# preon7/2019global

Measured on AMD Instinct MI355X. Metric: Mray/s + ms/frame at 1920x1080, depth 8; %HBM roofline, higher is better.
Workload: dtype f64

## Files before the change

2019global_amd/csrc/gi_wf.hip:

```cpp
#include <hip/hip_runtime.h>

#include <algorithm>
#include <cstdlib>
#include <mutex>
#include <type_traits>

#include "gi.h"
#include "gi_dev.h"
#include "gi_scene.h"

namespace gi {
namespace {

constexpr long long kWfTile = 8;

#ifndef GI_WF_MIN_WAVES_LDS
#define GI_WF_MIN_WAVES_LDS 4
#endif
#ifndef GI_WF_MIN_WAVES
#define GI_WF_MIN_WAVES 3
#endif
#ifndef GI_WF_TAKE
#define GI_WF_TAKE 16
#endif
constexpr size_t kWfSlotBytes = 9 * 256 * sizeof(double);

struct PathId {
    uint64_t key;
    unsigned smp;
    int b;
};
__device__ __forceinline__ void slot_put_u64(double* pl, int f, uint64_t v) { reinterpret_cast<uint64_t*>(pl)[f * 256] = v; }
__device__ __forceinline__ uint64_t slot_get_u64(const double* pl, int f) { return reinterpret_cast<const uint64_t*>(pl)[f * 256]; }

struct WFQ {
    double* r;
    uint2* id;
    long long cap;
};

template <bool ANY, bool PAIR, bool AXIS, bool SH, bool TRI, bool NST, typename NodeP, typename HotP>
__device__ __forceinline__ int wf_trace(float far_r, NodeP W, HotP H, V3 o, V3 d, double tmax, bool act, int* nst, double& t_out,
                                        uint32_t& nnode, uint32_t& nprim, uint32_t& nsteps, int skip = 254) {
    constexpr bool kSkip = std::is_same<NodeP, const XWNode*>::value;
    const F3 of = ray_org32(o, d, far_r);
    const F3 ivf = inv_dir(d);
    const int dmask = (d.x < 0 ? 1 : 0) | (d.y < 0 ? 2 : 0) | (d.z < 0 ? 4 : 0);
    double tb = tmax;
    float tbf = up32(tmax);
    int best = -1;
    uint64_t mlo = 0, mhi = 0;
    int node = 0, level = 0;
    bool raying = false;
    if (act) {
        uint32_t rm;
        if constexpr (kSkip) rm = children_mask<AXIS, true>(W, of, ivf, tbf, dmask, skip);
        else rm = children_mask<AXIS>(W, of, ivf, tbf, dmask);
        lvl_set<SH>(mlo, mhi, 0, rm);
        raying = rm != 0;
    }
    while (raying) {
        ++nsteps;
        const auto* nd = W + node;
        const uint32_t msk = lvl_get<SH>(mlo, mhi, level);
        const int kc = __builtin_ctz(msk);
        lvl_set<SH>(mlo, mhi, level, msk & (msk - 1));
        const int c = kc ^ dmask;
        bool keep = true;
        if (!ANY && !NST && best >= 0) {
            keep = child_hit(nd, c, of, ivf, tbf);
        }
        const int ch = nd->child[c];
        if (keep) {
            if (ch < 0) {
                const int cnt = nd->cnt[c];
                const auto* hp = H + ~ch;
                if constexpr (PAIR) {
                    for (int j = 0; j < cnt; j += 2) {
                        const bool two = j + 1 < cnt;
                        const XHotR r0 = load_hot(hp + j), r1 = load_hot(hp + (two ? j + 1 : j));
                        const double ta = x_prim_t<TRI>(r0.h, o, d, MX_TMIN);
                        const double tq = two ? x_prim_t<TRI>(r1.h, o, d, MX_TMIN) : INFINITY;
                        nprim += two ? 2 : 1;
                        if (ANY) {
                            if ((ta < tmax) | (tq < tmax)) {
                                best = ta < tmax ? r0.h.prim : r1.h.prim;
                                break;
                            }
                        } else {
                            const bool ua = (ta < tb) | ((ta == tb) & (r0.h.prim < best));
                            tb = ua ? ta : tb;
                            best = ua ? r0.h.prim : best;
                            const bool uq = (tq < tb) | ((tq == tb) & (r1.h.prim < best));
                            tb = uq ? tq : tb;
                            best = uq ? r1.h.prim : best;
                            tbf = up32(tb);
                        }
                    }
                } else {
                    XHotR cur = load_hot(hp);
                    for (int j = 0; j < cnt; ++j) {
                        const XHotR rec = cur;
                        if (j + 1 < cnt) cur = load_hot(hp + j + 1);
                        ++nprim;
                        const double t = x_prim_t<TRI>(rec.h, o, d, MX_TMIN);
                        if (ANY) {
                            if (t < tmax) { best = rec.h.prim; break; }
                        } else {
                            const bool u = (t < tb) | ((t == tb) & (rec.h.prim < best));
                            tb = u ? t : tb;
                            best = u ? rec.h.prim : best;
                            tbf = u ? up32(t) : tbf;
                        }
                    }
                }
            } else {
                ++nnode;
                uint32_t cm;
                if constexpr (kSkip) cm = children_mask<AXIS, true>(W + ch, of, ivf, tbf, dmask, skip);
                else cm = children_mask<AXIS>(W + ch, of, ivf, tbf, dmask);
                if (cm) {
                    node = ch;
                    ++level;
                    lvl_set<SH>(mlo, mhi, level, cm);
                    if (NST) nst[level * 256] = ch;
                }
            }
        }
        if (ANY && best >= 0) break;
        uint32_t rest = lvl_get<SH>(mlo, mhi, level);
        if (rest == 0 && level > 0) {
            if constexpr (NST) {
                const uint64_t lm = level >= 8 ? mlo : mlo & ((1ull << (8 * level)) - 1);
                const uint64_t hm = level <= 8 ? 0ull : mhi & ((1ull << (8 * (level - 8))) - 1);
                level = hm ? 8 + (63 - __clzll((long long)hm)) / 8 : lm ? (63 - __clzll((long long)lm)) / 8 : 0;
                rest = lvl_get<SH>(mlo, mhi, level);
                node = level == 0 ? 0 : nst[level * 256];
            } else {
                do {
                    --level;
                    node = level == 0 ? 0 : W[node].parent;
                    rest = lvl_get<SH>(mlo, mhi, level);
                } while (rest == 0 && level > 0);
            }
        }
        raying = rest != 0;
    }
    t_out = tb;
    return best;
}

#ifndef GI_XFLAT_CHUNK
#define GI_XFLAT_CHUNK 0
#endif
#ifndef GI_XFLAT_UNROLL
#define GI_XFLAT_UNROLL 4
#endif
#ifndef GI_XFLAT_LDS
#define GI_XFLAT_LDS 0
#endif
typedef uint32_t u32x8 __attribute__((ext_vector_type(8)));
__device__ __forceinline__ u32x8 flat_rec_uniform(const XFlatLeaf* tab, int k) {
#if GI_XFLAT_LDS
    const int4* q = reinterpret_cast<const int4*>(tab + k);
    const int4 a = q[0], b = q[1];
    return u32x8{(uint32_t)a.x, (uint32_t)a.y, (uint32_t)a.z, (uint32_t)a.w, (uint32_t)b.x, (uint32_t)b.y, (uint32_t)b.z, (uint32_t)b.w};
#else
    return *(const __attribute__((address_space(4))) u32x8*)(uintptr_t)(tab + k);
#endif
}
__device__ __forceinline__ uint32_t flat_pack(uint32_t off, int k, uint32_t w7) { return off | ((uint32_t)k << 16) | ((w7 & 0xFFu) << 24); }
__device__ __forceinline__ bool flat_hit(const XFlatLeaf* r, F3 no, F3 ivf, int sm, float tmax, uint32_t& pk, int k) {
    const int4* q = reinterpret_cast<const int4*>(r);
    const int4 a = q[0], b = q[1];
    const float lx = __int_as_float(a.x), ly = __int_as_float(a.y), lz = __int_as_float(a.z);
    const float hx = __int_as_float(a.w), hy = __int_as_float(b.x), hz = __int_as_float(b.y);
    const float nx = (sm & 1) ? hx : lx, fx = (sm & 1) ? lx : hx;
    const float ny = (sm & 2) ? hy : ly, fy = (sm & 2) ? ly : hy;
    const float nz = (sm & 4) ? hz : lz, fz = (sm & 4) ? lz : hz;
    const float tn = fmaxf(fmaxf(__builtin_fmaf(nx, ivf.x, no.x), __builtin_fmaf(ny, ivf.y, no.y)),
                           fmaxf(__builtin_fmaf(nz, ivf.z, no.z), 0.0f));
    const float tf = fminf(fminf(__builtin_fmaf(fx, ivf.x, no.x), __builtin_fmaf(fy, ivf.y, no.y)),
                           fminf(__builtin_fmaf(fz, ivf.z, no.z), tmax));
    pk = flat_pack((uint32_t)b.z, k, (uint32_t)b.w);
    return tn <= tf;
}
template <bool ANY, bool TRI>
__device__ __forceinline__ int wf_flat(float far_r, const XFlatLeaf* tab, int n, const XHot* H, V3 o, V3 d, double tmax, bool act,
                                       double& t_out, uint32_t& nnode, uint32_t& nprim, uint32_t& nsteps, int skip) {
    const F3 of = ray_org32(o, d, far_r);
    const F3 ivf = inv_dir(d);
    const F3 no = neg_oiv(of, ivf);
    const int sm = iv_signs(ivf);
    const bool sx = (sm & 1) != 0, sy = (sm & 2) != 0, sz = (sm & 4) != 0;
    double tb = tmax;
    float tbf = up32(tmax);
    int best = -1;
    const float tfa = act ? tbf : -1.0f;
    uint32_t m = 0, pk = 0;
    float tn1 = INFINITY, tn2 = INFINITY;
    auto step = [&](const u32x8 w, int k) {
        const float lx = __uint_as_float(w[0]), ly = __uint_as_float(w[1]), lz = __uint_as_float(w[2]);
        const float hx = __uint_as_float(w[3]), hy = __uint_as_float(w[4]), hz = __uint_as_float(w[5]);
        const float ax = __builtin_fmaf(lx, ivf.x, no.x), bx = __builtin_fmaf(hx, ivf.x, no.x);
        const float ay = __builtin_fmaf(ly, ivf.y, no.y), by = __builtin_fmaf(hy, ivf.y, no.y);
        const float az = __builtin_fmaf(lz, ivf.z, no.z), bz = __builtin_fmaf(hz, ivf.z, no.z);
        const float tn = fmaxf(fmaxf(sx ? bx : ax, sy ? by : ay), fmaxf(sz ? bz : az, 0.0f));
        const float tf = fminf(fminf(sx ? ax : bx, sy ? ay : by), fminf(sz ? az : bz, tfa));
        const bool hit = (tn <= tf) & ((int)((w[7] >> 16) & 0xFFu) != skip);
        const uint32_t pkk = flat_pack(w[6], k, w[7]);
        m |= hit ? 1u << k : 0u;
        if (ANY) {
            pk = hit ? pkk : pk;
        } else {
            const float th = hit ? tn : INFINITY;
            pk = th < tn1 ? pkk : pk;
            tn2 = __builtin_amdgcn_fmed3f(tn1, tn2, th);
            tn1 = fminf(tn1, th);
        }
    };
    int k0 = 0;
#if GI_XFLAT_CHUNK
    for (; k0 + 4 <= n; k0 += 4) {
        const u32x8 w0 = flat_rec_uniform(tab, k0), w1 = flat_rec_uniform(tab, k0 + 1);
        const u32x8 w2 = flat_rec_uniform(tab, k0 + 2), w3 = flat_rec_uniform(tab, k0 + 3);
        step(w0, k0);
        step(w1, k0 + 1);
        step(w2, k0 + 2);
        step(w3, k0 + 3);
    }
#pragma unroll 1
#else
#pragma unroll GI_XFLAT_UNROLL
#endif
    for (int k = k0; k < n; ++k) step(flat_rec_uniform(tab, k), k);
    if (act) nnode += (uint32_t)((n * (int)sizeof(XFlatLeaf) + 255) / 256);
    bool go = m != 0;
    if (go) m &= ~(1u << ((pk >> 16) & 0xFFu));
    while (go) {
        ++nsteps;
        const int cnt = (int)(pk >> 24);
        const XHot* hp = H + (pk & 0xFFFFu);
        for (int j = 0; j < cnt; j += 2) {
            const bool two = j + 1 < cnt;
            const XHotR r0 = load_hot(hp + j), r1 = load_hot(hp + (two ? j + 1 : j));
            const double ta = x_prim_t<TRI>(r0.h, o, d, MX_TMIN);
            const double tq = two ? x_prim_t<TRI>(r1.h, o, d, MX_TMIN) : INFINITY;
            nprim += two ? 2 : 1;
            if (ANY) {
                if ((ta < tmax) | (tq < tmax)) {
                    best = ta < tmax ? r0.h.prim : r1.h.prim;
                    break;
                }
            } else {
                const bool ua = (ta < tb) | ((ta == tb) & (r0.h.prim < best));
                tb = ua ? ta : tb;
                best = ua ? r0.h.prim : best;
                const bool uq = (tq < tb) | ((tq == tb) & (r1.h.prim < best));
                tb = uq ? tq : tb;
                best = uq ? r1.h.prim : best;
                tbf = up32(tb);
            }
        }
        go = false;
        if (ANY) {
            if (best < 0 && m != 0) {
                const int k = 31 - __builtin_clz(m);
                m &= ~(1u << k);
                const int4 b = reinterpret_cast<const int4*>(tab + k)[1];
                pk = flat_pack((uint32_t)b.z, k, (uint32_t)b.w);
                go = true;
            }
        } else {
            if (tn2 > tbf) m = 0;
            while (m != 0) {
                const int k = __builtin_ctz(m);
                m &= m - 1;
                if (flat_hit(tab + k, no, ivf, sm, tbf, pk, k)) {
                    go = true;
                    break;
                }
            }
        }
    }
    t_out = tb;
    return best;
}

struct WFArgs {
    const unsigned* list;
    const unsigned* n_list;
    double* part;
    unsigned* take;
    const unsigned* n_in;
    unsigned* n_out;
    unsigned long long u0, u1;
    unsigned s0, ns;
};

struct WFView {
    const XWNode* LW = nullptr;
    const XHot* LH = nullptr;
    const XPrim* XP = nullptr;
    const REnt* EN = nullptr;
    const XFlatLeaf* FT = nullptr;
    int* nst = nullptr;
    double* pl = nullptr;
};
template <bool LDS>
__device__ __forceinline__ WFView wf_stage(const DevScene& sc, int4* lds) {
    WFView v;
    v.XP = sc.xprims;
    v.EN = sc.ents;
    v.FT = sc.xflat;
    if constexpr (LDS) {
        const int nw = sc.n_xwnodes * (int)(sizeof(XWNode) / sizeof(int4));
        const int nh = sc.n_xhot * (int)(sizeof(XHot) / sizeof(int4));
        const int np = sc.n_xprims * (int)(sizeof(XPrim) / sizeof(int4));
        const int ne = sc.n_ents * (int)(sizeof(REnt) / sizeof(int4));
        const int nf = GI_XFLAT_LDS ? sc.n_xflat * (int)(sizeof(XFlatLeaf) / sizeof(int4)) : 0;
        const int4* gw = reinterpret_cast<const int4*>(sc.xwnodes);
        const int4* gh = reinterpret_cast<const int4*>(sc.xhot);
        const int4* gp = reinterpret_cast<const int4*>(sc.xprims);
        const int4* ge = reinterpret_cast<const int4*>(sc.ents);
        const int4* gf = reinterpret_cast<const int4*>(sc.xflat);
        for (int i = threadIdx.x; i < nw; i += blockDim.x) lds[i] = gw[i];
        for (int i = threadIdx.x; i < nh; i += blockDim.x) lds[nw + i] = gh[i];
        for (int i = threadIdx.x; i < np; i += blockDim.x) lds[nw + nh + i] = gp[i];
        for (int i = threadIdx.x; i < ne; i += blockDim.x) lds[nw + nh + np + i] = ge[i];
        for (int i = threadIdx.x; i < nf; i += blockDim.x) lds[nw + nh + np + ne + i] = gf[i];
        __syncthreads();
        v.LW = reinterpret_cast<const XWNode*>(lds);
        v.LH = reinterpret_cast<const XHot*>(lds + nw);
        v.XP = reinterpret_cast<const XPrim*>(lds + nw + nh);
        v.EN = reinterpret_cast<const REnt*>(lds + nw + nh + np);
        if (GI_XFLAT_LDS) v.FT = reinterpret_cast<const XFlatLeaf*>(lds + nw + nh + np + ne);
        v.pl = reinterpret_cast<double*>(lds + nw + nh + np + ne + nf) + threadIdx.x;
    } else {
        v.nst = reinterpret_cast<int*>(lds) + threadIdx.x;
        v.pl = reinterpret_cast<double*>(reinterpret_cast<int*>(lds) + 16 * 256) + threadIdx.x;
    }
    return v;
}

__device__ __forceinline__ V3 wf_primary(const CamDev& cam, const TileMap& m, unsigned ps, int spp, uint64_t seed,
                                         unsigned li, unsigned smp, long long& idx, uint64_t& key) {
    int x = 0, y = 0;
    slot_pixel(m, (long long)(ps >> 6), (int)(ps & 63), idx, x, y);
    y += m.y0;
    if (spp > 1) idx = (long long)li;
    key = mx_key(seed, (uint64_t)y * (uint64_t)m.w + (uint64_t)x);
    double jx = 0.0, jy = 0.0;
    if (spp > 1) {
        jx = mx_u01k(key, smp, 0xFFFF, 0);
        jy = mx_u01k(key, smp, 0xFFFF, 1);
    }
    return primary_dir(cam, (double)x + jx, (double)y + jy);
}
__device__ __forceinline__ bool wf_primary_misses(const DevScene& sc, const CamDev& cam, V3 d0) {
    const F3 iv0 = f3(__builtin_amdgcn_rcpf((float)d0.x), __builtin_amdgcn_rcpf((float)d0.y), __builtin_amdgcn_rcpf((float)d0.z));
    return !root_hit(sc, ray_org32(cam.pos, d0, ray_far_r(sc, cam.pos)), iv0);
}
__device__ __forceinline__ void wf_store(double* part, double* rgb, uint8_t* rgb8, int spp, long long idx, unsigned smp, V3 L) {
    if (spp > 1) {
        double* q = part + 3 * ((size_t)idx * (size_t)spp + (size_t)smp);
        q[0] = L.x; q[1] = L.y; q[2] = L.z;
    } else {
        const double c0 = smin((0.0 + L.x) / 1.0, 1.0), c1 = smin((0.0 + L.y) / 1.0, 1.0), c2 = smin((0.0 + L.z) / 1.0, 1.0);
        if (rgb) { rgb[3 * idx] = c0; rgb[3 * idx + 1] = c1; rgb[3 * idx + 2] = c2; }
        if (rgb8) quantize(c0, c1, c2, rgb8 + 3 * idx);
    }
}

struct WFSegStats {
    uint64_t it_c = 0, ln_c = 0, it_s = 0, ln_s = 0, segs = 0, live = 0, iters = 0;
    uint64_t cyc_c = 0, cyc_s = 0, cyc_sh = 0, cyc_ref = 0, cyc_all = 0;
};
__device__ __forceinline__ void wf_wave_steps(uint32_t n, uint64_t& it, uint64_t& ln) {
    uint32_t mx = n, sm = n;
    for (int off = 32; off > 0; off >>= 1) {
        mx = max(mx, (uint32_t)__shfl_xor(mx, off));
        sm += __shfl_xor(sm, off);
    }
    if ((threadIdx.x & 63) == 0) { it += mx; ln += sm; }
}
template <bool ANY, bool LDS, bool SH, bool TRI, bool CN, bool FLAT>
__device__ __forceinline__ int x_query(const DevScene& sc, const WFView& v, float far_r, const V3& o, const V3& d, double tmax,
                                       bool act, double& t_out, uint32_t& nnode, uint32_t& nprim, uint32_t& st_steps, int skip) {
    if constexpr (FLAT) return wf_flat<ANY, TRI>(far_r, v.FT, sc.n_xflat, v.LH, o, d, tmax, act, t_out, nnode, nprim, st_steps, skip);
    else if constexpr (LDS) return wf_trace<ANY, true, false, SH, TRI, false>(far_r, v.LW, v.LH, o, d, tmax, act, v.nst, t_out, nnode, nprim, st_steps, skip);
    else if constexpr (CN) return wf_trace<ANY, false, false, SH, TRI, true>(far_r, sc.xcnodes, sc.xhot, o, d, tmax, act, v.nst, t_out, nnode, nprim, st_steps);
    else return wf_trace<ANY, false, false, SH, TRI, true>(far_r, sc.xwnodes, sc.xhot, o, d, tmax, act, v.nst, t_out, nnode, nprim, st_steps, skip);
}
__device__ __forceinline__ int x_own_plane(int pg, const V3& pn, const V3& dir, double skip_cos) {
    return (pg < 254 && fabs(dot(dir, pn)) >= skip_cos) ? pg : 254;
}
struct XHitFrame { V3 P, Ld, pn; double ldist; int pg; };
__device__ __forceinline__ XHitFrame x_hit_frame(const WFView& v, const V3& light, const V3& o, const V3& d, bool hit, int best, double t) {
    XHitFrame h{o, v3(0, 0, 1), v3(0, 0, 1), 0.0, 254};
    if (hit) {
        h.P = o + t * d;
        const V3 lv = light - h.P;
        h.ldist = gsqrt(dot(lv, lv));
        h.Ld = normalize(lv);
        const XPrim& px = v.XP[best];
        h.pg = px.pad[0] < 254 ? px.pad[0] : 254;
        h.pn = ld3(px.n);
    }
    return h;
}

template <bool STATS, bool LDS, bool SH, bool TRI, bool CN, bool FLAT, typename KeyF>
__device__ __forceinline__ bool x_segment(const DevScene& sc, const WFView& v, const V3& light, int depth, bool no_shadow, bool act,
                                          const KeyF& id_of, V3& o, V3& d, V3& L, V3& T,
                                          uint32_t& nnode, uint32_t& nprim, uint32_t& nrays, WFSegStats& ws,
                                          double skip_cos = 2.0, int* splane = nullptr, float far_r = INFINITY) {
    uint32_t st_steps = 0;
    uint64_t c0 = STATS ? clock64() : 0;
    bool occl = false;
    double tbest = INFINITY;
    const int skip_c = splane ? *splane : 254;
    const int best = x_query<false, LDS, SH, TRI, CN, FLAT>(sc, v, far_r, o, d, INFINITY, act, tbest, nnode, nprim, st_steps, skip_c);
    if (act) ++nrays;
    if (STATS) {
        wf_wave_steps(st_steps, ws.it_c, ws.ln_c);
        st_steps = 0;
        const uint64_t c1 = clock64();
        ws.cyc_c += c1 - c0;
        c0 = c1;
    }
    const bool hit = act && best >= 0;
    const XHitFrame h = x_hit_frame(v, light, o, d, hit, best, tbest);
    const V3 &P = h.P, &Ld = h.Ld;
    if (!no_shadow) {
        double tdummy;
        const int skip_s = x_own_plane(h.pg, h.pn, Ld, skip_cos);
        occl = x_query<true, LDS, SH, TRI, CN, FLAT>(sc, v, INFINITY, P, Ld, h.ldist, hit, tdummy, nnode, nprim, st_steps, skip_s) >= 0;
        if (STATS) wf_wave_steps(st_steps, ws.it_s, ws.ln_s);
    }
    if (STATS) {
        const uint64_t c1 = clock64();
        ws.cyc_s += c1 - c0;
        c0 = c1;
    }
    {
        L = v3(v.pl[0], v.pl[256], v.pl[512]);
        T = v3(v.pl[768], v.pl[1024], v.pl[1280]);
    }
    bool cont = false;
    if (hit) {
        ++nrays;
        const XPrim& p = v.XP[best];
        V3 N = (TRI || p.kind == 0) ? ld3(p.n) : normalize(P - ld3(p.a));
        N = dot(d, N) < 0 ? N : -N;
        const REnt& e = v.EN[p.ent];
        int32_t tu, tv;
        x_texcoord<TRI>(sc, e, P, tu, tv);
        const V3 tc = texel(ld3(e.color), tu, tv);
        const V3 la = tc * e.shader[0];
        V3 loc = la;
        if (!occl) {
            const V3 ldf = (smax(0.0, dot(N, Ld)) * (tc * 0.5)) * e.shader[1];
            const V3 bis = normalize(normalize(-d) + Ld);
            const double spw = mx_pow(smax(0.0, dot(N, bis)), e.spec_pow);
            const V3 ls = v3(spw, spw, spw) * e.shader[2];
            loc = (la + ldf) + ls;
        }
        L = L + vmul(T, v3(smin(loc.x, 1.0), smin(loc.y, 1.0), smin(loc.z, 1.0)));
        const PathId id = id_of();
        const uint64_t key = id.key;
        const unsigned smp = id.smp;
        const int b = id.b;
        if (b != depth - 1) {
            if (e.refl > 0.0 && mx_u01k(key, smp, b, 4) < e.refl) {
                d = normalize(d - N * (2.0 * dot(d, N)));
                cont = true;
            } else {
                T = vmul(T, tc * 0.5);
                if (!((T.x == 0.0) & (T.y == 0.0) & (T.z == 0.0))) {
                    double sx, sy, r2;
                    mx_disk(mx_u01k(key, smp, b, 2), mx_u01k(key, smp, b, 3), sx, sy, r2);
                    const double sz = gsqrt(1.0 - r2);
                    const double sg = N.z >= 0.0 ? 1.0 : -1.0;
                    const double aa = -1.0 / (sg + N.z);
                    const double bb = N.x * N.y * aa;
                    const V3 bt1 = v3(1.0 + sg * N.x * N.x * aa, sg * bb, -sg * N.x);
                    const V3 bt2 = v3(bb, sg + N.y * N.y * aa, -N.y);
                    d = normalize((bt1 * sx + bt2 * sy) + N * sz);
                    cont = true;
                }
            }
            o = P;
        }
        if (cont) {
            v.pl[0] = L.x; v.pl[256] = L.y; v.pl[512] = L.z;
            v.pl[768] = T.x; v.pl[1024] = T.y; v.pl[1280] = T.z;
            if (splane) *splane = x_own_plane(h.pg, h.pn, d, skip_cos);
        }
    }
    if (STATS) ws.cyc_sh += clock64() - c0;
    return cont;
}

template <bool STATS, bool LDS, bool W4, bool SH, bool TRI, bool CN, bool FLAT>
__global__ __launch_bounds__(256, (LDS && W4) ? GI_WF_MIN_WAVES_LDS : GI_WF_MIN_WAVES) void k_wf_bounce(
    DevScene sc, CamDev cam, V3 light, TileMap m, int spp, int depth, uint64_t seed, int b, double* rgb, uint8_t* rgb8,
    unsigned long long* stats, WFArgs a, WFQ qin, WFQ qout, int xflags) {
    unsigned n_in;
    if (b == 0) {
        const unsigned long long tot = (unsigned long long)*a.n_list * (unsigned long long)a.ns;
        n_in = (unsigned)(min(tot, a.u1) > a.u0 ? min(tot, a.u1) - a.u0 : 0ull);
    } else {
        n_in = *a.n_in;
    }
    if (*(volatile unsigned*)a.take >= n_in) return;
    extern __shared__ int4 lds_dyn[];
    const WFView v = wf_stage<LDS>(sc, lds_dyn);
    const bool no_shadow = (xflags & XF_NO_SHADOW) != 0;
    const int lane = threadIdx.x & 63;
    uint32_t nnode = 0, nprim = 0, nrays = 0, nres = 0, npx = 0;
    const long long qc = qin.cap, oc = qout.cap;
    const unsigned take = (unsigned)max(1u, min((unsigned)GI_WF_TAKE, n_in / (64u * 8u * (gridDim.x * (blockDim.x >> 6)))));
    unsigned base = 0, left = 0;
    for (;;) {
        if (left == 0) {
            if (lane == 0) base = atomicAdd(a.take, 64u * take);
            base = __shfl(base, 0);
            left = take;
        }
        if (base >= n_in) break;
        const unsigned j = base + (unsigned)lane;
        base += 64u;
        --left;
        bool act = j < n_in;
        unsigned li = 0, smp = 0;
        V3 o = cam.pos, d = v3(1, 0, 0), L = v3(0, 0, 0), T = v3(1, 1, 1);
        long long idx = -1;
        uint64_t key = 0;
        if (act) {
            if (b == 0) {
                const unsigned long long u = a.u0 + j;
                if (u < (1ull << 32)) {
                    li = (unsigned)u / a.ns;
                    smp = a.s0 + ((unsigned)u - li * a.ns);
                } else {
                    li = (unsigned)(u / (unsigned long long)a.ns);
                    smp = a.s0 + (unsigned)(u - (unsigned long long)li * (unsigned long long)a.ns);
                }
            } else {
                const uint2 id = qin.id[j];
                li = id.x;
                smp = id.y;
                const double* r = qin.r + j;
                o = v3(r[0], r[qc], r[2 * qc]);
                d = v3(r[3 * qc], r[4 * qc], r[5 * qc]);
                L = v3(r[6 * qc], r[7 * qc], r[8 * qc]);
                T = v3(r[9 * qc], r[10 * qc], r[11 * qc]);
            }
            const V3 d0 = wf_primary(cam, m, a.list[li], spp, seed, li, smp, idx, key);
            if (b == 0) {
                if (smp == 0) ++npx;
                if (wf_primary_misses(sc, cam, d0)) {
                    ++nrays;
                    ++nres;
                    act = false;
                    wf_store(a.part, rgb, rgb8, spp, idx, smp, v3(0, 0, 0));
                } else {
                    d = normalize(d0);
                }
            }
            v.pl[0] = L.x; v.pl[256] = L.y; v.pl[512] = L.z;
            v.pl[768] = T.x; v.pl[1024] = T.y; v.pl[1280] = T.z;
        }
        WFSegStats ws;
        const double skip_cos = x_skip_cos(sc, cam.pos);
        const float far_r = ray_far_r(sc, cam.pos);
        int splane = 254;
        const bool cont = x_segment<false, LDS, SH, TRI, CN, FLAT>(sc, v, light, depth, no_shadow, act, [&] { return PathId{key, smp, b}; }, o, d, L, T,
                                                             nnode, nprim, nrays, ws, skip_cos, &splane, far_r);
        const unsigned long long mc = __ballot(cont);
        if (mc) {
            const int leader = __ffsll((long long)mc) - 1;
            unsigned ob = 0;
            if (lane == leader) ob = atomicAdd(a.n_out, (unsigned)__popcll(mc));
            ob = __shfl(ob, leader);
            if (cont) {
                const unsigned k = ob + (unsigned)__popcll(mc & ((1ull << lane) - 1));
                qout.id[k] = make_uint2(li, smp);
                double* r = qout.r + k;
                r[0] = o.x; r[oc] = o.y; r[2 * oc] = o.z;
                r[3 * oc] = d.x; r[4 * oc] = d.y; r[5 * oc] = d.z;
                r[6 * oc] = L.x; r[7 * oc] = L.y; r[8 * oc] = L.z;
                r[9 * oc] = T.x; r[10 * oc] = T.y; r[11 * oc] = T.z;
            }
        }
        if (act && !cont) wf_store(a.part, rgb, rgb8, spp, idx, smp, L);
    }
    if (STATS) {
        wave_add_stats(stats, nrays, nnode, nprim, npx);
        uint64_t r = nres;
        for (int off = 32; off > 0; off >>= 1) r += __shfl_xor(r, off);
        if (lane == 0 && r) atomicAdd(stats + GI_STAT_X_RESOLVED, (unsigned long long)r);
    }
}

#ifndef GI_SEG_BURST
#define GI_SEG_BURST 16
#endif
#ifndef GI_SEG_TAKE
#define GI_SEG_TAKE 2
#endif
#ifndef GI_SEG_TAKE_TRI
#define GI_SEG_TAKE_TRI 1
#endif
template <bool STATS, bool LDS, bool W4, bool SH, bool TRI, bool CN, bool FLAT>
__global__ __launch_bounds__(256, (LDS && W4) ? GI_WF_MIN_WAVES_LDS : GI_WF_MIN_WAVES) void k_seg(
    DevScene sc, CamDev cam, V3 light, TileMap m, int spp, int depth, uint64_t seed, double* rgb, uint8_t* rgb8,
    unsigned long long* stats, WFArgs a, int xflags) {
    extern __shared__ int4 lds_dyn[];
    const WFView v = wf_stage<LDS>(sc, lds_dyn);
    const bool no_shadow = (xflags & XF_NO_SHADOW) != 0;
    const int lane = threadIdx.x & 63;
    const unsigned long long total = (unsigned long long)*a.n_list * (unsigned long long)a.ns;
    constexpr long long kTake = (LDS && TRI) ? GI_SEG_TAKE_TRI : GI_SEG_TAKE;
    const unsigned long long n_waves = (unsigned long long)gridDim.x * (blockDim.x >> 6);
    const unsigned long long run = 64ull * (unsigned long long)max(1ll, min(kTake, (long long)(total / (64ull * 8ull * n_waves))));
    uint32_t nnode = 0, nprim = 0, nrays = 0, nres = 0, npx = 0;
    unsigned long long cur = 0, cur_end = 0;
    bool exhausted = false;
    bool live = false;
    unsigned li = 0, smp = 0;
    long long idx = -1;
    uint64_t key = 0;
    V3 o = cam.pos, d = v3(1, 0, 0), L = v3(0, 0, 0), T = v3(1, 1, 1);
    int splane = 254;
    const double skip_cos = x_skip_cos(sc, cam.pos);
    const float far_r = ray_far_r(sc, cam.pos);
    WFSegStats ws;
    const uint64_t t_begin = STATS ? clock64() : 0;
    for (;;) {
        if (STATS && lane == 0) ++ws.iters;
        const uint64_t t_ref = STATS ? clock64() : 0;
        for (int burst = 0; burst < GI_SEG_BURST; ++burst) {
            const unsigned long long m_need = __ballot(!live);
            if (m_need == 0 || (exhausted && cur >= cur_end)) break;
            const unsigned rank = (unsigned)__popcll(m_need & ((1ull << lane) - 1));
            const unsigned n_need = (unsigned)__popcll(m_need);
            unsigned long long u = ~0ull;
            const unsigned long long avail = cur_end - cur;
            if (n_need > avail && !exhausted) {
                unsigned long long nb = 0;
                if (lane == 0) nb = atomicAdd(reinterpret_cast<unsigned long long*>(a.take), run);
                nb = __shfl(nb, 0);
                if (nb >= total) {
                    exhausted = true;
                    if (!live && rank < avail) u = cur + rank;
                    cur = cur_end;
                } else {
                    const unsigned long long ne = min(total, nb + run);
                    if (!live) {
                        if (rank < avail) u = cur + rank;
                        else if (nb + (rank - avail) < ne) u = nb + (rank - avail);
                    }
                    cur = min(ne, nb + (n_need - avail));
                    cur_end = ne;
                    if (ne == total) exhausted = true;
                }
            } else {
                if (!live && rank < avail) u = cur + rank;
                cur += min((unsigned long long)n_need, avail);
            }
            unsigned li_u = 0, smp_u = 0;
            if (u != ~0ull) {
                if (u < (1ull << 32)) {
                    li_u = (unsigned)u / a.ns;
                    smp_u = a.s0 + ((unsigned)u - li_u * a.ns);
                } else {
                    li_u = (unsigned)(u / (unsigned long long)a.ns);
                    smp_u = a.s0 + (unsigned)(u - (unsigned long long)li_u * (unsigned long long)a.ns);
                }
            }
            if (!live && u != ~0ull) {
                li = li_u;
                smp = smp_u;
                const unsigned ps = a.list[li];
                const V3 d0 = wf_primary(cam, m, ps, spp, seed, li, smp, idx, key);
                if (smp == 0) ++npx;
                if (wf_primary_misses(sc, cam, d0)) {
                    ++nrays;
                    ++nres;
                    wf_store(a.part, rgb, rgb8, spp, idx, smp, v3(0, 0, 0));
                } else {
                    live = true;
                    o = cam.pos;
                    d = normalize(d0);
                    splane = 254;
                    L = v3(0, 0, 0);
                    T = v3(1, 1, 1);
                    v.pl[0] = 0.0; v.pl[256] = 0.0; v.pl[512] = 0.0;
                    v.pl[768] = 1.0; v.pl[1024] = 1.0; v.pl[1280] = 1.0;
                    slot_put_u64(v.pl, 6, key);
                    slot_put_u64(v.pl, 7, (uint64_t)(uint32_t)idx | ((uint64_t)smp << 32));
                    slot_put_u64(v.pl, 8, 0ull);
                }
            }
        }
        if (STATS) ws.cyc_ref += clock64() - t_ref;
        if (__ballot(live) == 0) {
            if (exhausted && cur >= cur_end) break;
            continue;
        }
        if (STATS) {
            const unsigned long long ml = __ballot(live);
            if (lane == 0) { ++ws.segs; ws.live += __popcll(ml); }
        }
        const bool cont = x_segment<STATS, LDS, SH, TRI, CN, FLAT>(
            sc, v, light, depth, no_shadow, live,
            [&] { return PathId{slot_get_u64(v.pl, 6), (unsigned)(slot_get_u64(v.pl, 7) >> 32), (int)slot_get_u64(v.pl, 8)}; },
            o, d, L, T, nnode, nprim, nrays, ws, skip_cos, &splane, far_r);
        if (live) {
            if (cont) {
                slot_put_u64(v.pl, 8, slot_get_u64(v.pl, 8) + 1);
            } else {
                const uint64_t is = slot_get_u64(v.pl, 7);
                wf_store(a.part, rgb, rgb8, spp, (long long)(uint32_t)is, (unsigned)(is >> 32), L);
                live = false;
            }
        }
    }
    if (STATS && lane == 0) {
        atomicAdd(stats + GI_STAT_X_ITERS, (unsigned long long)ws.iters);
        atomicAdd(stats + GI_STAT_X_HANDLE, (unsigned long long)ws.segs);
        atomicAdd(stats + GI_STAT_X_HLANES, (unsigned long long)ws.live);
        atomicAdd(stats + GI_STAT_X_IT_LEAF, (unsigned long long)ws.it_c);
        atomicAdd(stats + GI_STAT_X_LN_LEAF, (unsigned long long)ws.ln_c);
        atomicAdd(stats + GI_STAT_X_IT_NODE, (unsigned long long)ws.it_s);
        atomicAdd(stats + GI_STAT_X_LN_NODE, (unsigned long long)ws.ln_s);
        atomicAdd(stats + GI_STAT_X_CYC_TRAV, (unsigned long long)(ws.cyc_c + ws.cyc_s));
        atomicAdd(stats + GI_STAT_X_IT_RS, (unsigned long long)ws.cyc_c);
        atomicAdd(stats + GI_STAT_X_CYC_HIT, (unsigned long long)ws.cyc_sh);
        atomicAdd(stats + GI_STAT_X_CYC_NEXT, (unsigned long long)ws.cyc_ref);
        atomicAdd(stats + GI_STAT_X_CYC_ALL, (unsigned long long)(clock64() - t_begin));
    }
    if (STATS) {
        wave_add_stats(stats, nrays, nnode, nprim, npx);
        uint64_t r = nres;
        for (int off = 32; off > 0; off >>= 1) r += __shfl_xor(r, off);
        if (lane == 0 && r) atomicAdd(stats + GI_STAT_X_RESOLVED, (unsigned long long)r);
    }
}

template <bool LDS, bool W4, bool SH, bool TRI, bool CN, bool FLAT>
__global__ __launch_bounds__(256, (LDS && W4) ? GI_WF_MIN_WAVES_LDS : GI_WF_MIN_WAVES) void k_x_query_kat(
    DevScene sc, V3 cam_pos, int n, const double* recs, int32_t* oi, double* od) {
    extern __shared__ int4 lds_dyn[];
    const WFView v = wf_stage<LDS>(sc, lds_dyn);
    const long long i = (long long)blockIdx.x * 256 + threadIdx.x;
    const bool act = i < (long long)n;
    const double skip_cos = x_skip_cos(sc, cam_pos);
    const float far_r = ray_far_r(sc, cam_pos);
    V3 o = v3(0, 0, 0), d = v3(1, 0, 0), light = v3(0, 0, 0), d2 = v3(1, 0, 0);
    if (act) {
        const double* q = recs + 12 * i;
        o = v3(q[0], q[1], q[2]);
        d = v3(q[3], q[4], q[5]);
        light = v3(q[6], q[7], q[8]);
        d2 = v3(q[9], q[10], q[11]);
    }
    uint32_t nnode = 0, nprim = 0, st_steps = 0;
    double t1 = INFINITY;
    const int p1 = x_query<false, LDS, SH, TRI, CN, FLAT>(sc, v, far_r, o, d, INFINITY, act, t1, nnode, nprim, st_steps, 254);
    const bool hit = act && p1 >= 0;
    const XHitFrame h = x_hit_frame(v, light, o, d, hit, p1, t1);
    double tdummy;
    const int skip_s = x_own_plane(h.pg, h.pn, h.Ld, skip_cos);
    const int sb = x_query<true, LDS, SH, TRI, CN, FLAT>(sc, v, INFINITY, h.P, h.Ld, h.ldist, hit, tdummy, nnode, nprim, st_steps, skip_s);
    const int skip2 = x_own_plane(h.pg, h.pn, d2, skip_cos);
    double t2 = INFINITY;
    const int p2 = x_query<false, LDS, SH, TRI, CN, FLAT>(sc, v, far_r, h.P, d2, INFINITY, hit, t2, nnode, nprim, st_steps, skip2);
    if (act) {
        oi[5 * i] = p1 >= 0 ? p1 : -1;
        oi[5 * i + 1] = hit ? (sb >= 0 ? 1 : 0) : -1;
        oi[5 * i + 2] = skip_s;
        oi[5 * i + 3] = (hit && p2 >= 0) ? p2 : -1;
        oi[5 * i + 4] = skip2;
        od[2 * i] = p1 >= 0 ? t1 : INFINITY;
        od[2 * i + 1] = (hit && p2 >= 0) ? t2 : INFINITY;
    }
    if (i == 0) od[2 * (long long)n] = skip_cos;
}

template <bool ANY, bool LDS, bool W4, bool SH, bool TRI, bool CN, bool FLAT>
__global__ __launch_bounds__(256, (LDS && W4) ? GI_WF_MIN_WAVES_LDS : GI_WF_MIN_WAVES) void k_cast(DevScene sc, CastIO io) {
    extern __shared__ int4 lds_dyn[];
    const WFView v = wf_stage<LDS>(sc, lds_dyn);
    const int lane = threadIdx.x & 63;
    const long long stride = 64ll * (long long)gridDim.x * (long long)(blockDim.x >> 6);
    for (long long base = 64ll * ((long long)blockIdx.x * (blockDim.x >> 6) + (threadIdx.x >> 6)); base < io.n; base += stride) {
        const long long i = base + lane;
        const bool in = i < io.n;
        V3 o = v3(0, 0, 0), d = v3(1, 0, 0);
        double tmax = INFINITY;
        bool act = false;
        if (in) {
            const double2* q = reinterpret_cast<const double2*>(io.rays) + 4 * i;
            const double2 q0 = q[0], q1 = q[1], q2 = q[2], q3 = q[3];
            const V3 ro = v3(q0.x, q0.y, q1.x), rd = v3(q1.y, q2.x, q2.y);
            const bool fin = __builtin_isfinite(ro.x) & __builtin_isfinite(ro.y) & __builtin_isfinite(ro.z) &
                             __builtin_isfinite(rd.x) & __builtin_isfinite(rd.y) & __builtin_isfinite(rd.z);
            const bool nz = (rd.x != 0.0) | (rd.y != 0.0) | (rd.z != 0.0);
            act = fin & nz & (q3.x > MX_TMIN);
            if (act) {
                o = ro;
                d = rd;
                tmax = q3.x;
            }
        }
        uint32_t nnode = 0, nprim = 0, nsteps = 0;
        double tb = INFINITY;
        const int best = x_query<ANY, LDS, SH, TRI, CN, FLAT>(sc, v, sc.x_far_r, o, d, tmax, act, tb, nnode, nprim, nsteps, 254);
        const bool hit = act && best >= 0;
        if constexpr (ANY) {
            if (in) io.occl[i] = hit ? 1 : 0;
        } else {
            if (in) {
                if (io.t) io.t[i] = hit ? tb : INFINITY;
                if (io.prim) io.prim[i] = hit ? best : -1;
                if (io.ent || io.nrm) {
                    int ent = -1;
                    V3 N = v3(0, 0, 0);
                    if (hit) {
                        const XPrim& p = v.XP[best];
                        ent = p.ent;
                        const V3 P = o + tb * d;
                        N = (TRI || p.kind == 0) ? ld3(p.n) : normalize(P - ld3(p.a));
                        N = dot(d, N) < 0 ? N : -N;
                    }
                    if (io.ent) io.ent[i] = ent;
                    if (io.nrm) {
                        double* q = io.nrm + 3 * i;
                        q[0] = N.x; q[1] = N.y; q[2] = N.z;
                    }
                }
            }
        }
    }
}

__host__ __device__ inline long long aov_batches(int cols, int rows) { return ((long long)cols * (long long)rows + 63) / 64; }
__device__ __forceinline__ bool aov_pixel(int cols, int rows, long long b, int lane, int& px, int& py) {
    const long long i = 64 * b + lane;
    if (i < (1ll << 32)) {
        const unsigned q = (unsigned)i / (unsigned)cols;
        py = (int)q;
        px = (int)((unsigned)i - q * (unsigned)cols);
    } else {
        const long long q = i / (long long)cols;
        py = (int)q;
        px = (int)(i - q * (long long)cols);
    }
    return i < (long long)cols * (long long)rows;
}

template <bool LDS, bool W4, bool SH, bool TRI, bool CN, bool FLAT>
__global__ __launch_bounds__(256, (LDS && W4) ? GI_WF_MIN_WAVES_LDS : GI_WF_MIN_WAVES) void k_aov(DevScene sc, CamDev cam, AovIO io) {
    extern __shared__ int4 lds_dyn[];
    const WFView v = wf_stage<LDS>(sc, lds_dyn);
    const int lane = threadIdx.x & 63;
    const float far_r = ray_far_r(sc, cam.pos);
    const long long n_batches = aov_batches(io.cols, io.rows);
    const long long stride = (long long)gridDim.x * (long long)(blockDim.x >> 6);
    const bool want_tex = io.alb || io.uv;
    for (long long b = (long long)blockIdx.x * (blockDim.x >> 6) + (threadIdx.x >> 6); b < n_batches; b += stride) {
        int px = 0, py = 0;
        const bool in = aov_pixel(io.cols, io.rows, b, lane, px, py);
        const V3 o = cam.pos;
        V3 d = v3(1, 0, 0);
        bool act = false;
        if (in) {
            const V3 d0 = primary_dir(cam, (double)(io.x0 + px), (double)(io.y0 + py));
            if (!wf_primary_misses(sc, cam, d0)) {
                act = true;
                d = normalize(d0);
            }
        }
        uint32_t nnode = 0, nprim = 0, nsteps = 0;
        double tb = INFINITY;
        const int best = x_query<false, LDS, SH, TRI, CN, FLAT>(sc, v, far_r, o, d, INFINITY, act, tb, nnode, nprim, nsteps, 254);
        const bool hit = act && best >= 0;
        if (in) {
            const long long i = (long long)py * (long long)io.cols + (long long)px;
            int ent = -1, tu = 0, tv = 0;
            V3 N = v3(0, 0, 0), tc = v3(0, 0, 0);
            if (hit) {
                const XPrim& p = v.XP[best];
                ent = p.ent;
                const V3 P = o + tb * d;
                N = (TRI || p.kind == 0) ? ld3(p.n) : normalize(P - ld3(p.a));
                N = dot(d, N) < 0 ? N : -N;
                if (want_tex) {
                    const REnt& e = v.EN[p.ent];
                    x_texcoord<TRI>(sc, e, P, tu, tv);
                    tc = texel(ld3(e.color), tu, tv);
                }
            }
            if (io.t) io.t[i] = hit ? tb : INFINITY;
            if (io.prim) io.prim[i] = hit ? best : -1;
            if (io.ent) io.ent[i] = ent;
            if (io.nrm) {
                double* q = io.nrm + 3 * i;
                q[0] = N.x; q[1] = N.y; q[2] = N.z;
            }
            if (io.alb) {
                double* q = io.alb + 3 * i;
                q[0] = tc.x; q[1] = tc.y; q[2] = tc.z;
            }
            if (io.uv) {
                int32_t* q = io.uv + 2 * i;
                q[0] = tu; q[1] = tv;
            }
        }
    }
}

__global__ __launch_bounds__(256) void k_cam_rays(CamDev cam, int x0, int y0, int cols, int rows, double* rays) {
    const long long n_batches = aov_batches(cols, rows);
    const long long stride = (long long)gridDim.x * (long long)(blockDim.x >> 6);
    const int lane = threadIdx.x & 63;
    for (long long b = (long long)blockIdx.x * (blockDim.x >> 6) + (threadIdx.x >> 6); b < n_batches; b += stride) {
        int px = 0, py = 0;
        if (!aov_pixel(cols, rows, b, lane, px, py)) continue;
        const V3 d = normalize(primary_dir(cam, (double)(x0 + px), (double)(y0 + py)));
        double2* q = reinterpret_cast<double2*>(rays) + 4 * (64 * b + lane);
        q[0] = make_double2(cam.pos.x, cam.pos.y);
        q[1] = make_double2(cam.pos.z, d.x);
        q[2] = make_double2(d.y, d.z);
        q[3] = make_double2(INFINITY, 0.0);
    }
}

}

size_t wf_slot_bytes() { return kWfSlotBytes; }
size_t wf_scene_lds_bytes(const DevScene& sc) { return (size_t)sc.x_lds_bytes + (GI_XFLAT_LDS ? (size_t)sc.n_xflat * sizeof(XFlatLeaf) : 0); }

template <typename F>
void wf_dispatch(const DevScene& sc, XVariant var, bool flat, bool stats, F&& f) {
    if (var.lds && flat && sc.x_flat)
        with_bools([&](auto S, auto W) { f(XTag<S.value, true, W.value, true, W.value, false, true>{}); }, stats, var.w4);
    else if (var.lds)
        with_bools([&](auto S, auto W, auto H) { f(XTag<S.value, true, W.value, H.value, W.value, false, false>{}); },
                   stats, var.w4, sc.x_max_depth <= 7);
    else
        with_bools([&](auto S, auto T, auto C) { f(XTag<S.value, false, false, false, T.value, C.value, false>{}); },
                   stats, sc.x_tri_only != 0, sc.xcnodes != nullptr);
}
template <typename V>
constexpr auto seg_kernel(V) { return &k_seg<V::stats, V::lds, V::w4, V::sh, V::tri, V::cn, V::flat>; }
template <typename V>
constexpr auto bounce_kernel(V) { return &k_wf_bounce<V::stats, V::lds, V::w4, V::sh, V::tri, V::cn, V::flat>; }

template <bool ANY, typename V>
constexpr auto cast_kernel(V) { return &k_cast<ANY, V::lds, V::w4, V::sh, V::tri, V::cn, V::flat>; }

template <typename V>
constexpr auto aov_kernel(V) { return &k_aov<V::lds, V::w4, V::sh, V::tri, V::cn, V::flat>; }

hipError_t wf_occupancy(const DevScene& sc, XVariant var, bool flat, size_t lds_bytes, int form, int* per_cu) {
    hipError_t e = hipSuccess;
    wf_dispatch(sc, var, flat, false, [&](auto V) {
        const void* f = form == 5   ? reinterpret_cast<const void*>(aov_kernel(V))
                        : form == 4 ? reinterpret_cast<const void*>(cast_kernel<true>(V))
                        : form == 3 ? reinterpret_cast<const void*>(cast_kernel<false>(V))
                        : form == 2 ? reinterpret_cast<const void*>(seg_kernel(V))
                                    : reinterpret_cast<const void*>(bounce_kernel(V));
        e = hipOccupancyMaxActiveBlocksPerMultiprocessor(per_cu, f, 256, lds_bytes);
    });
    return e;
}

hipError_t launch_wf(const DevScene& sc, XVariant var, size_t lds_bytes, int resident, int form, const CamDev& cam, V3 light,
                     int w, int h, int y0, const gi_opts& o, double* rgb, uint8_t* rgb8, const XScratch& xs,
                     const unsigned* n_list_dev, unsigned long long* stats, int xflags, hipStream_t stream,
                     hipEvent_t ev_begin, hipEvent_t ev_end) {
    const TileMap m = make_map(w, h, o.shard_count, o.shard_index, y0);
    const int depth = o.depth;
    const int s0 = o.sample_end > 0 ? o.sample_begin : 0, s1 = o.sample_end > 0 ? o.sample_end : o.spp;
    const dim3 grid((unsigned)std::max(1, resident)), block(256);
    hipError_t e = hipSuccess;
    const bool flat = (xflags & XF_NO_FLAT) == 0;
    if (form == 2) {
        WFArgs a{};
        a.list = xs.list;
        a.n_list = n_list_dev;
        a.part = xs.part;
        a.take = xs.wcnt;
        a.s0 = (unsigned)s0;
        a.ns = (unsigned)(s1 - s0);
        if (ev_begin) (void)hipEventRecord(ev_begin, stream);
        wf_dispatch(sc, var, flat, stats != nullptr, [&](auto V) {
            hipLaunchKernelGGL(seg_kernel(V), grid, block, lds_bytes, stream, sc, cam, light, m, o.spp, depth, o.seed, rgb, rgb8, stats, a, xflags);
        });
        if (ev_end) (void)hipEventRecord(ev_end, stream);
        return hipGetLastError();
    }
    const unsigned long long units = (unsigned long long)m.n_local * (unsigned long long)(kWfTile * kWfTile) *
                                     (unsigned long long)(s1 - s0);
    if (ev_begin) (void)hipEventRecord(ev_begin, stream);
    for (unsigned long long u0 = 0; u0 < units; u0 += (unsigned long long)xs.wcap) {
        e = hipMemsetAsync(xs.wcnt, 0, 2 * (size_t)depth * sizeof(unsigned), stream);
        if (e != hipSuccess) return e;
        for (int b = 0; b < depth; ++b) {
            WFArgs a;
            a.list = xs.list;
            a.n_list = n_list_dev;
            a.part = xs.part;
            a.take = xs.wcnt + 2 * b;
            a.n_in = b > 0 ? xs.wcnt + 2 * (b - 1) + 1 : nullptr;
            a.n_out = xs.wcnt + 2 * b + 1;
            a.u0 = u0;
            a.u1 = std::min(units, u0 + (unsigned long long)xs.wcap);
            a.s0 = (unsigned)s0;
            a.ns = (unsigned)(s1 - s0);
            WFQ qin, qout;
            qin.cap = qout.cap = xs.wcap;
            qin.r = xs.wq[(b + 1) & 1];
            qin.id = reinterpret_cast<uint2*>(xs.wid[(b + 1) & 1]);
            qout.r = xs.wq[b & 1];
            qout.id = reinterpret_cast<uint2*>(xs.wid[b & 1]);
            wf_dispatch(sc, var, flat, stats != nullptr, [&](auto V) {
                hipLaunchKernelGGL(bounce_kernel(V), grid, block, lds_bytes, stream, sc, cam, light, m, o.spp, depth, o.seed, b, rgb, rgb8, stats, a, qin, qout, xflags);
            });
        }
    }
    if (ev_end) (void)hipEventRecord(ev_end, stream);
    return hipGetLastError();
}

hipError_t launch_x_query_kat(const DevScene& sc, XVariant var, bool flat, size_t lds_bytes, V3 cam_pos, int n,
                              const double* recs, int32_t* oi, double* od, hipStream_t stream) {
    if (n <= 0) return hipSuccess;
    const dim3 grid((unsigned)(((long long)n + 255) / 256)), block(256);
    wf_dispatch(sc, var, flat, false, [&](auto V) {
        using T = decltype(V);
        hipLaunchKernelGGL((k_x_query_kat<T::lds, T::w4, T::sh, T::tri, T::cn, T::flat>), grid, block, lds_bytes, stream, sc, cam_pos, n, recs, oi, od);
    });
    return hipGetLastError();
}

hipError_t launch_cast(const DevScene& sc, XVariant var, bool flat, size_t lds_bytes, int resident, bool any, const CastIO& io,
                       hipStream_t stream) {
    if (io.n <= 0) return hipSuccess;
    const long long want = (io.n + 255) / 256;
    const dim3 grid((unsigned)std::max<long long>(1, std::min<long long>(want, resident))), block(256);
    wf_dispatch(sc, var, flat, false, [&](auto V) {
        if (any) hipLaunchKernelGGL(cast_kernel<true>(V), grid, block, lds_bytes, stream, sc, io);
        else hipLaunchKernelGGL(cast_kernel<false>(V), grid, block, lds_bytes, stream, sc, io);
    });
    return hipGetLastError();
}

hipError_t launch_aov_kernel(const DevScene& sc, XVariant var, bool flat, size_t lds_bytes, int resident, const CamDev& cam,
                             const AovIO& io, hipStream_t stream) {
    if (io.cols <= 0 || io.rows <= 0) return hipSuccess;
    const long long want = (aov_batches(io.cols, io.rows) + 3) / 4;
    const dim3 grid((unsigned)std::max<long long>(1, std::min<long long>(want, resident))), block(256);
    wf_dispatch(sc, var, flat, false, [&](auto V) {
        hipLaunchKernelGGL(aov_kernel(V), grid, block, lds_bytes, stream, sc, cam, io);
    });
    return hipGetLastError();
}

hipError_t launch_cam_rays(const CamDev& cam, int x0, int y0, int cols, int rows, double* rays, hipStream_t stream) {
    if (cols <= 0 || rows <= 0) return hipSuccess;
    const long long want = ((long long)cols * (long long)rows + 255) / 256;
    const dim3 grid((unsigned)std::min<long long>(want, 2048)), block(256);
    hipLaunchKernelGGL(k_cam_rays, grid, block, 0, stream, cam, x0, y0, cols, rows, rays);
    return hipGetLastError();
}

void wf_variant(const DevScene& sc, XVariant var, bool flat, int32_t out[6]) {
    wf_dispatch(sc, var, flat, false, [&](auto V) {
        out[0] = V.lds; out[1] = V.w4; out[2] = V.sh; out[3] = V.tri; out[4] = V.cn; out[5] = V.flat;
    });
}

}
```

Before: 31410.

## Pack flat-leaf hit masks via ballot shift and integer sort keys with LDS pk table

The flat-leaf traversal builds its hit mask by shifting in wave ballots through v_addc carry, which reverses the bit order. It tracks the nearest two hits as packed integer keys (tn bits with the leaf index in the low 5 bits) instead of float tn plus a per-step pk select. The packed offset/count words for each leaf are precomputed into LDS at kernel start, so descending to a leaf reads one word instead of reloading the record. This trims per-leaf VALU work and selects, at the cost of extra LDS space and staging, inline asm, and a small loss of tn precision in the early-out threshold.

```diff
diff --git a/2019global_amd/csrc/gi_wf.hip b/2019global_amd/csrc/gi_wf.hip
--- a/2019global_amd/csrc/gi_wf.hip
+++ b/2019global_amd/csrc/gi_wf.hip
@@ -150,26 +150,25 @@
     return best;
 }
 
-#ifndef GI_XFLAT_CHUNK
-#define GI_XFLAT_CHUNK 0
-#endif
-#ifndef GI_XFLAT_UNROLL
-#define GI_XFLAT_UNROLL 4
-#endif
-#ifndef GI_XFLAT_LDS
-#define GI_XFLAT_LDS 0
-#endif
+constexpr size_t kFlatPkBytes = GI_XFLAT_MAX * sizeof(uint32_t);
 typedef uint32_t u32x8 __attribute__((ext_vector_type(8)));
 __device__ __forceinline__ u32x8 flat_rec_uniform(const XFlatLeaf* tab, int k) {
-#if GI_XFLAT_LDS
-    const int4* q = reinterpret_cast<const int4*>(tab + k);
-    const int4 a = q[0], b = q[1];
-    return u32x8{(uint32_t)a.x, (uint32_t)a.y, (uint32_t)a.z, (uint32_t)a.w, (uint32_t)b.x, (uint32_t)b.y, (uint32_t)b.z, (uint32_t)b.w};
-#else
     return *(const __attribute__((address_space(4))) u32x8*)(uintptr_t)(tab + k);
-#endif
 }
 __device__ __forceinline__ uint32_t flat_pack(uint32_t off, int k, uint32_t w7) { return off | ((uint32_t)k << 16) | ((w7 & 0xFFu) << 24); }
+__device__ __forceinline__ uint32_t flat_shift_in(uint32_t m, unsigned long long hm) {
+    uint32_t r;
+    asm("v_addc_co_u32 %0, vcc, %1, %1, %2" : "=v"(r) : "v"(m), "s"(hm) : "vcc");
+    return r;
+}
+__device__ __forceinline__ int flat_key(float tn, int k) {
+    int r;
+    asm("v_bfi_b32 %0, 31, %1, %2" : "=v"(r) : "s"(k), "v"(tn));
+    return r;
+}
+__device__ __forceinline__ int flat_med3(int a, int b, int c) { return max(min(a, b), min(max(a, b), c)); }
+__device__ __forceinline__ float flat_key_floor(int e) { return __int_as_float(e & ~31); }
+__device__ __forceinline__ uint32_t flat_pk_of(const uint32_t* pkw, int k) { return pkw[k]; }
 __device__ __forceinline__ bool flat_hit(const XFlatLeaf* r, F3 no, F3 ivf, int sm, float tmax, uint32_t& pk, int k) {
     const int4* q = reinterpret_cast<const int4*>(r);
     const int4 a = q[0], b = q[1];
@@ -186,7 +185,7 @@
     return tn <= tf;
 }
 template <bool ANY, bool TRI>
-__device__ __forceinline__ int wf_flat(float far_r, const XFlatLeaf* tab, int n, const XHot* H, V3 o, V3 d, double tmax, bool act,
+__device__ __forceinline__ int wf_flat(float far_r, const XFlatLeaf* tab, const uint32_t* pkw, int n, const XHot* H, V3 o, V3 d, double tmax, bool act,
                                        double& t_out, uint32_t& nnode, uint32_t& nprim, uint32_t& nsteps, int skip) {
     const F3 of = ray_org32(o, d, far_r);
     const F3 ivf = inv_dir(d);
@@ -196,9 +195,10 @@
     double tb = tmax;
     float tbf = up32(tmax);
     int best = -1;
-    const float tfa = act ? tbf : -1.0f;
+    const float tfa = __builtin_canonicalizef(act ? tbf : -1.0f);
+    constexpr int kNone = 0x7F800000;
     uint32_t m = 0, pk = 0;
-    float tn1 = INFINITY, tn2 = INFINITY;
+    int e1 = kNone, e2 = kNone;
     auto step = [&](const u32x8 w, int k) {
         const float lx = __uint_as_float(w[0]), ly = __uint_as_float(w[1]), lz = __uint_as_float(w[2]);
         const float hx = __uint_as_float(w[3]), hy = __uint_as_float(w[4]), hz = __uint_as_float(w[5]);
@@ -207,20 +207,16 @@
         const float az = __builtin_fmaf(lz, ivf.z, no.z), bz = __builtin_fmaf(hz, ivf.z, no.z);
         const float tn = fmaxf(fmaxf(sx ? bx : ax, sy ? by : ay), fmaxf(sz ? bz : az, 0.0f));
         const float tf = fminf(fminf(sx ? ax : bx, sy ? ay : by), fminf(sz ? az : bz, tfa));
-        const bool hit = (tn <= tf) & ((int)((w[7] >> 16) & 0xFFu) != skip);
-        const uint32_t pkk = flat_pack(w[6], k, w[7]);
-        m |= hit ? 1u << k : 0u;
-        if (ANY) {
-            pk = hit ? pkk : pk;
-        } else {
-            const float th = hit ? tn : INFINITY;
-            pk = th < tn1 ? pkk : pk;
-            tn2 = __builtin_amdgcn_fmed3f(tn1, tn2, th);
-            tn1 = fminf(tn1, th);
+        const bool in = tn <= tf, other = (int)((w[7] >> 16) & 0xFFu) != skip;
+        m = flat_shift_in(m, __builtin_amdgcn_ballot_w64(in) & __builtin_amdgcn_ballot_w64(other));
+        if (!ANY) {
+            const int key = flat_key(tn, k);
+            const int eh = (in & other) ? key : kNone;
+            e2 = flat_med3(e1, e2, eh);
+            e1 = min(e1, eh);
         }
     };
     int k0 = 0;
-#if GI_XFLAT_CHUNK
     for (; k0 + 4 <= n; k0 += 4) {
         const u32x8 w0 = flat_rec_uniform(tab, k0), w1 = flat_rec_uniform(tab, k0 + 1);
         const u32x8 w2 = flat_rec_uniform(tab, k0 + 2), w3 = flat_rec_uniform(tab, k0 + 3);
@@ -230,13 +226,14 @@
         step(w3, k0 + 3);
     }
 #pragma unroll 1
-#else
-#pragma unroll GI_XFLAT_UNROLL
-#endif
     for (int k = k0; k < n; ++k) step(flat_rec_uniform(tab, k), k);
     if (act) nnode += (uint32_t)((n * (int)sizeof(XFlatLeaf) + 255) / 256);
     bool go = m != 0;
-    if (go) m &= ~(1u << ((pk >> 16) & 0xFFu));
+    if (go) {
+        const int bit = (ANY || e1 == kNone) ? __builtin_ctz(m) : n - 1 - (e1 & 31);
+        m &= ~(1u << bit);
+        pk = flat_pk_of(pkw, n - 1 - bit);
+    }
     while (go) {
         ++nsteps;
         const int cnt = (int)(pk >> 24);
@@ -265,17 +262,17 @@
         go = false;
         if (ANY) {
             if (best < 0 && m != 0) {
-                const int k = 31 - __builtin_clz(m);
-                m &= ~(1u << k);
-                const int4 b = reinterpret_cast<const int4*>(tab + k)[1];
-                pk = flat_pack((uint32_t)b.z, k, (uint32_t)b.w);
+                const int bit = __builtin_ctz(m);
+                m &= m - 1;
+                pk = flat_pk_of(pkw, n - 1 - bit);
                 go = true;
             }
         } else {
-            if (tn2 > tbf) m = 0;
+            if (flat_key_floor(e2) > tbf) m = 0;
             while (m != 0) {
-                const int k = __builtin_ctz(m);
-                m &= m - 1;
+                const int bit = 31 - __builtin_clz(m);
+                m &= ~(1u << bit);
+                const int k = n - 1 - bit;
                 if (flat_hit(tab + k, no, ivf, sm, tbf, pk, k)) {
                     go = true;
                     break;
@@ -304,10 +301,11 @@
     const XPrim* XP = nullptr;
     const REnt* EN = nullptr;
     const XFlatLeaf* FT = nullptr;
+    const uint32_t* FP = nullptr;
     int* nst = nullptr;
     double* pl = nullptr;
 };
-template <bool LDS>
+template <bool LDS, bool FLAT = false>
 __device__ __forceinline__ WFView wf_stage(const DevScene& sc, int4* lds) {
     WFView v;
     v.XP = sc.xprims;
@@ -318,24 +316,26 @@
         const int nh = sc.n_xhot * (int)(sizeof(XHot) / sizeof(int4));
         const int np = sc.n_xprims * (int)(sizeof(XPrim) / sizeof(int4));
         const int ne = sc.n_ents * (int)(sizeof(REnt) / sizeof(int4));
-        const int nf = GI_XFLAT_LDS ? sc.n_xflat * (int)(sizeof(XFlatLeaf) / sizeof(int4)) : 0;
         const int4* gw = reinterpret_cast<const int4*>(sc.xwnodes);
         const int4* gh = reinterpret_cast<const int4*>(sc.xhot);
         const int4* gp = reinterpret_cast<const int4*>(sc.xprims);
         const int4* ge = reinterpret_cast<const int4*>(sc.ents);
-        const int4* gf = reinterpret_cast<const int4*>(sc.xflat);
         for (int i = threadIdx.x; i < nw; i += blockDim.x) lds[i] = gw[i];
         for (int i = threadIdx.x; i < nh; i += blockDim.x) lds[nw + i] = gh[i];
         for (int i = threadIdx.x; i < np; i += blockDim.x) lds[nw + nh + i] = gp[i];
         for (int i = threadIdx.x; i < ne; i += blockDim.x) lds[nw + nh + np + i] = ge[i];
-        for (int i = threadIdx.x; i < nf; i += blockDim.x) lds[nw + nh + np + ne + i] = gf[i];
+        constexpr int nk = FLAT ? (int)(kFlatPkBytes / sizeof(int4)) : 0;
+        if constexpr (FLAT) {
+            uint32_t* pkw = reinterpret_cast<uint32_t*>(lds + nw + nh + np + ne);
+            for (int i = threadIdx.x; i < sc.n_xflat; i += blockDim.x) pkw[i] = flat_pack((uint32_t)sc.xflat[i].off, i, (uint32_t)sc.xflat[i].cnt);
+            v.FP = pkw;
+        }
         __syncthreads();
         v.LW = reinterpret_cast<const XWNode*>(lds);
         v.LH = reinterpret_cast<const XHot*>(lds + nw);
         v.XP = reinterpret_cast<const XPrim*>(lds + nw + nh);
         v.EN = reinterpret_cast<const REnt*>(lds + nw + nh + np);
-        if (GI_XFLAT_LDS) v.FT = reinterpret_cast<const XFlatLeaf*>(lds + nw + nh + np + ne);
-        v.pl = reinterpret_cast<double*>(lds + nw + nh + np + ne + nf) + threadIdx.x;
+        v.pl = reinterpret_cast<double*>(lds + nw + nh + np + ne + nk) + threadIdx.x;
     } else {
         v.nst = reinterpret_cast<int*>(lds) + threadIdx.x;
         v.pl = reinterpret_cast<double*>(reinterpret_cast<int*>(lds) + 16 * 256) + threadIdx.x;
@@ -387,7 +387,7 @@
 template <bool ANY, bool LDS, bool SH, bool TRI, bool CN, bool FLAT>
 __device__ __forceinline__ int x_query(const DevScene& sc, const WFView& v, float far_r, const V3& o, const V3& d, double tmax,
                                        bool act, double& t_out, uint32_t& nnode, uint32_t& nprim, uint32_t& st_steps, int skip) {
-    if constexpr (FLAT) return wf_flat<ANY, TRI>(far_r, v.FT, sc.n_xflat, v.LH, o, d, tmax, act, t_out, nnode, nprim, st_steps, skip);
+    if constexpr (FLAT) return wf_flat<ANY, TRI>(far_r, v.FT, v.FP, sc.n_xflat, v.LH, o, d, tmax, act, t_out, nnode, nprim, st_steps, skip);
     else if constexpr (LDS) return wf_trace<ANY, true, false, SH, TRI, false>(far_r, v.LW, v.LH, o, d, tmax, act, v.nst, t_out, nnode, nprim, st_steps, skip);
     else if constexpr (CN) return wf_trace<ANY, false, false, SH, TRI, true>(far_r, sc.xcnodes, sc.xhot, o, d, tmax, act, v.nst, t_out, nnode, nprim, st_steps);
     else return wf_trace<ANY, false, false, SH, TRI, true>(far_r, sc.xwnodes, sc.xhot, o, d, tmax, act, v.nst, t_out, nnode, nprim, st_steps, skip);
@@ -515,7 +515,7 @@
     }
     if (*(volatile unsigned*)a.take >= n_in) return;
     extern __shared__ int4 lds_dyn[];
-    const WFView v = wf_stage<LDS>(sc, lds_dyn);
+    const WFView v = wf_stage<LDS, FLAT>(sc, lds_dyn);
     const bool no_shadow = (xflags & XF_NO_SHADOW) != 0;
     const int lane = threadIdx.x & 63;
     uint32_t nnode = 0, nprim = 0, nrays = 0, nres = 0, npx = 0;
@@ -618,7 +618,7 @@
     DevScene sc, CamDev cam, V3 light, TileMap m, int spp, int depth, uint64_t seed, double* rgb, uint8_t* rgb8,
     unsigned long long* stats, WFArgs a, int xflags) {
     extern __shared__ int4 lds_dyn[];
-    const WFView v = wf_stage<LDS>(sc, lds_dyn);
+    const WFView v = wf_stage<LDS, FLAT>(sc, lds_dyn);
     const bool no_shadow = (xflags & XF_NO_SHADOW) != 0;
     const int lane = threadIdx.x & 63;
     const unsigned long long total = (unsigned long long)*a.n_list * (unsigned long long)a.ns;
@@ -754,7 +754,7 @@
 __global__ __launch_bounds__(256, (LDS && W4) ? GI_WF_MIN_WAVES_LDS : GI_WF_MIN_WAVES) void k_x_query_kat(
     DevScene sc, V3 cam_pos, int n, const double* recs, int32_t* oi, double* od) {
     extern __shared__ int4 lds_dyn[];
-    const WFView v = wf_stage<LDS>(sc, lds_dyn);
+    const WFView v = wf_stage<LDS, FLAT>(sc, lds_dyn);
     const long long i = (long long)blockIdx.x * 256 + threadIdx.x;
     const bool act = i < (long long)n;
     const double skip_cos = x_skip_cos(sc, cam_pos);
@@ -793,7 +793,7 @@
 template <bool ANY, bool LDS, bool W4, bool SH, bool TRI, bool CN, bool FLAT>
 __global__ __launch_bounds__(256, (LDS && W4) ? GI_WF_MIN_WAVES_LDS : GI_WF_MIN_WAVES) void k_cast(DevScene sc, CastIO io) {
     extern __shared__ int4 lds_dyn[];
-    const WFView v = wf_stage<LDS>(sc, lds_dyn);
+    const WFView v = wf_stage<LDS, FLAT>(sc, lds_dyn);
     const int lane = threadIdx.x & 63;
     const long long stride = 64ll * (long long)gridDim.x * (long long)(blockDim.x >> 6);
     for (long long base = 64ll * ((long long)blockIdx.x * (blockDim.x >> 6) + (threadIdx.x >> 6)); base < io.n; base += stride) {
@@ -865,7 +865,7 @@
 template <bool LDS, bool W4, bool SH, bool TRI, bool CN, bool FLAT>
 __global__ __launch_bounds__(256, (LDS && W4) ? GI_WF_MIN_WAVES_LDS : GI_WF_MIN_WAVES) void k_aov(DevScene sc, CamDev cam, AovIO io) {
     extern __shared__ int4 lds_dyn[];
-    const WFView v = wf_stage<LDS>(sc, lds_dyn);
+    const WFView v = wf_stage<LDS, FLAT>(sc, lds_dyn);
     const int lane = threadIdx.x & 63;
     const float far_r = ray_far_r(sc, cam.pos);
     const long long n_batches = aov_batches(io.cols, io.rows);
@@ -942,7 +942,7 @@
 }
 
 size_t wf_slot_bytes() { return kWfSlotBytes; }
-size_t wf_scene_lds_bytes(const DevScene& sc) { return (size_t)sc.x_lds_bytes + (GI_XFLAT_LDS ? (size_t)sc.n_xflat * sizeof(XFlatLeaf) : 0); }
+size_t wf_scene_lds_bytes(const DevScene& sc) { return (size_t)sc.x_lds_bytes + (sc.x_flat ? kFlatPkBytes : 0); }
 
 template <typename F>
 void wf_dispatch(const DevScene& sc, XVariant var, bool flat, bool stats, F&& f) {
```

Measured after the change: 32380, median of 6. 1.03x the previous value.
